# alexandre01/deepsvg

Hardware: AMD Instinct MI355X
Metric: SVG icons/sec (train step) hierarchical_ordered d=256 (higher is better)
Workload: dtype bf16; 1 GPU; hierarchical_ordered (Hierarchical, use_vae=False) G=8 S=30 d_model=256 ff=512 H=8 L=4x4; full train step = forward + SVGLoss + backward + grad-clip 1.0 + AdamW; dropout 0.1; global_batch=512, batch_per_gpu=512, parallelism=dp1, hip_graph=True, encoder_layout=packed (valid tokens only, exact)

## Files before the change

### deepsvg_amd/functional.py

```python
import math
import contextlib
import functools
import os

import torch

from . import ops

FFN_BWD_FUSED = os.environ.get("DSVG_FFN_BWD_FUSED", "0") != "0"
FFN_MIN_ROWS = int(os.environ.get("DSVG_FFN_MIN_ROWS", "16384"))
ATTN_MIN_ROWS = int(os.environ.get("DSVG_ATTN_MIN_ROWS", "16384"))
FFN_BWD_ORDER = os.environ.get("DSVG_FFN_BWD_ORDER", "1") != "0"
FFN_BWD_MASKED = int(os.environ.get("DSVG_FFN_BWD_MASKED", "0"))

GROUP_WGRAD = os.environ.get("DSVG_GROUP_WGRAD", "1") != "0"
BCAST_MASKED = os.environ.get("DSVG_BCAST_MASKED", "1") != "0"
LN_BWD_MASKED = os.environ.get("DSVG_LN_BWD_MASKED", "1") != "0"
DEFER_MORE = os.environ.get("DSVG_DEFER_MORE", "1") != "0"
STACK_GROUP = os.environ.get("DSVG_STACK_GROUP", "1") != "0"
STACK_GROUP_SLICES = int(os.environ.get("DSVG_STACK_GROUP_SLICES", "8"))
GS_BWD_DG = os.environ.get("DSVG_GS_BWD_DG", "1") != "0"
HEAD_KPAD = os.environ.get("DSVG_HEAD_KPAD", "1") != "0"
COND_GRAD_SHARED = os.environ.get("DSVG_COND_GRAD_SHARED", "1") != "0"
GS_STACK = os.environ.get("DSVG_GS_STACK", "1") != "0"
ATTN_BWD_OUTPROJ = os.environ.get("DSVG_ATTN_BWD_OUTPROJ", "1") != "0"
_ATTN_VALU = os.environ.get("DSVG_ATTN_VALU") is not None
_ATTN_MFMA_MIN_S = int(os.environ.get("DSVG_ATTN_MFMA_MIN_S", "2"))
ATTN_BWD_DX = os.environ.get("DSVG_ATTN_BWD_DX", "0") != "0"
ATTN_BWD_DX_MIN_ROWS = int(os.environ.get("DSVG_ATTN_BWD_DX_MIN_ROWS", "8192"))
GS_REMAINDER = int(os.environ.get("DSVG_GS_REMAINDER", "512"))
SEQ_ROUND = 2048
HEAD_FUSED = os.environ.get("DSVG_HEAD_FUSED", "0") != "0"

_NULL_CTX = contextlib.nullcontext()

class Runtime:

    def __init__(self, dtype=torch.float32, seed=None, store=None, training=False, defer=False):
        self.dtype = dtype
        self.defer = bool(defer)
        self.seed = seed
        self.store = store
        self.training = training
        self.masked = {}
        self.last_layer_gs = False
        self.stack_group = None
        self.cond_grad = {}

    def cond_grad_block(self, z, rows):
        if not COND_GRAD_SHARED or z is None or z.dim() != 2 or z.stride(1) != 1 or z.dtype != torch.bfloat16:
            return None
        w, ld = z.shape[1], z.stride(0)
        if ld <= w or ld % w or w % 8 or w > 512:
            return None
        i = (z.storage_offset() % ld) // w
        if (z.storage_offset() % ld) % w:
            return None
        base = z.data_ptr() - i * w * z.element_size()
        key = (base, rows, ld)
        buf = self.cond_grad.get(key)
        if buf is None:
            if len(self.cond_grad) > 8:
                self.cond_grad.clear()
            buf = self.cond_grad[key] = torch.empty((rows, ld), dtype=z.dtype, device=z.device)
        return buf[:, i * w:(i + 1) * w]

# ... 680 lines not shown
                elif ctx.needs_input_grad[3]:
                    dz = ops.gemm(dg, rt.w(wg), b_kc=False)
            nsl = STACK_GROUP_SLICES if (STACK_GROUP and GROUP_WGRAD and rt.defer) else 8
            gb = (lambda w_: nsl * -(-w_.shape[0] // 128) * -(-w_.shape[1] // 128)) if GROUP_WGRAD else (lambda w_: None)
            keep = rt.stack_group_begin() if (STACK_GROUP and GROUP_WGRAD and rt.defer) else None
            with (rt.grouping() if keep is None else _NULL_CTX):
                with ops.tag("ffn"):
                    dw2, db2 = _wbgrad(rt, w2, b2, dym, h, gb(w2))
                    dw1, db1 = _wbgrad(rt, w1, b1, dpre, xn2, gb(w1))
                if z is not None and wg is not None:
                    dwg, dbg = _wbgrad(rt, wg, bg, dg, z, gb(wg))
                dwo, dbo = _wbgrad(rt, wo, bo, dx1m, ao, gb(wo))
                dwin, dbin = _wbgrad(rt, win, bin_, dqkv, xn1, gb(win))
            if keep is not None:
                keep += [dym, h, dpre, xn2, dx1m, ao, dqkv, xn1, dg, z]
                if ctx.first_in_stack:
                    rt.stack_group_end()
            return (None, dx, None, dz, None, None, None, None, None, None,
                    dn1w, dn1b, dwin, dbin, dwo, dbo, dn2w, dn2b, dw1, db1, dw2, db2, dwg, dbg, None, None, None, None, None,
                    None, None, None)
        if ctx.ffn_fused:
            pb, b1f, w2p = rt.store.ffn(w1)[1:]
            T = x1.shape[0]
            with ops.tag("ffn"):
                g2p = torch.empty((256, 512), dtype=torch.float32, device=x1.device)
                g1p = torch.empty((512, 256), dtype=torch.float32, device=x1.device)
                db1p = torch.empty(512, dtype=torch.float32, device=x1.device)
                db2 = rt.grad_out(b2)
                s2, s1 = ops.split_k_for(256, 512, T), ops.split_k_for(512, 256, T)

                def wgrad2(dym, hp):
                    with rt.deferring():
                        if s2 > 1:
                            ops.gemm(dym, hp, a_kc=False, b_kc=False, out=g2p, split_k=s2, rowsum=db2)
                        else:
                            ops.gemm(dym, hp, a_kc=False, b_kc=False, out=g2p)
                            ops.colsum(dym, out=db2)

                def wgrad1(dpre, xh):
                    with rt.deferring():
                        if s1 > 1:
                            ops.gemm(dpre, xh, a_kc=False, b_kc=False, out=g1p, split_k=s1, rowsum=db1p)
                        else:
                            ops.gemm(dpre, xh, a_kc=False, b_kc=False, out=g1p)
                            ops.colsum(dpre, out=db1p)

                if h is None:
                    dx1, hp, dpre, xh, dym = ops.ffn_bwd(x1, dx2, pb, b1f, 1e-5, p, s0 + 3, s0 + 4, rt.seed)
                    wgrad2(dym, hp)
                    wgrad1(dpre, xh)
                else:
                    hp, xh = h, xn2
                    dym = dx2_masked if dx2_masked is not None else ops.drop_apply(dx2, p, s0 + 4, rt.seed)
                    if FFN_BWD_ORDER:
                        wgrad2(dym, hp)
                    dpre = ops.gemm(dym, w2p, b_kc=False, gate=hp, gate_scale=inv_keep)
                    if FFN_BWD_ORDER:
                        wgrad1(dpre, xh)
                    if FFN_BWD_MASKED == 1 or (FFN_BWD_MASKED == 2 and z is None and p > 0):
                        dx1, dx1m = ops.ffn_bwd_dx(dpre, x1, dx2, pb, masked=(p, s0 + 1, rt.seed))
                    else:
                        dx1 = ops.ffn_bwd_dx(dpre, x1, dx2, pb)
                    if not FFN_BWD_ORDER:
                        wgrad2(dym, hp)
                        wgrad1(dpre, xh)
                dw1, db1, dw2 = rt.grad_out(w1), rt.grad_out(b1), rt.grad_out(w2)
                dn2w, dn2b = rt.grad_out(n2w), rt.grad_out(n2b)
                fin = (g1p, db1p, g2p, w1.detach(), n2w.detach(), n2b.detach(), dw1.detach(), db1.detach(), dw2.detach(),
                       dn2w.detach(), dn2b.detach())
                if rt.defer:
                    ops.ffn_wgrad_finish_deferred(*fin)
                else:
                    ops.ffn_wgrad_finish(*fin)
            del hp, dpre, xh, dym
        else:
            with ops.tag("ffn"):
                dx2m = dx2_masked if dx2_masked is not None else ops.drop_apply(dx2, p, s0 + 4, rt.seed)
                dw2, db2 = _wbgrad(rt, w2, b2, dx2m, h)
                dh = ops.gemm(dx2m, rt.w(w2), b_kc=False, gate=h, gate_scale=inv_keep)
                dw1, db1 = _wbgrad(rt, w1, b1, dh, xn2)
                dxn2 = ops.gemm(dh, rt.w(w1), b_kc=False)
                with rt.deferring():
                    dx1, dn2w, dn2b = ops.layernorm_bwd(dxn2, x1, mean2, rstd2, n2w.detach(), res=dx2,
                                                        dgamma=rt.grad_out(n2w), dbeta=rt.grad_out(n2b))
            del dx2m
        dz = dl = dwg = dbg = dwg2 = dbg2 = None
        if l is not None:
            dg2 = ops.bcast_add_bwd(dx1, n_seq, S, p, s0 + 5, rt.seed)
            dwg2, dbg2 = _wbgrad(rt, wg2, bg2, dg2, l)
            if ctx.needs_input_grad[4]:
                dl = ops.gemm(dg2, rt.w(wg2), b_kc=False)
        if z is not None:
            vec = dx1.dtype == torch.bfloat16 and dx1.is_contiguous() and dx1.shape[1] % 8 == 0 and dx1.shape[1] <= 512
            dg_out = rt.cond_grad_block(z, n_seq_full) if (wg is None and vec and dx1.data_ptr() % 16 == 0) else None
            if BCAST_MASKED and dx1m is None and p > 0 and vec and n_seq * S <= dx1.shape[0] <= n_seq_full * S:
                dg, dx1m = ops.bcast_add_bwd(dx1, n_seq, S, p, s0 + 2, rt.seed, n_seq_out=n_seq_full, mask_site=s0 + 1, out=dg_out)
            else:
                dg = ops.bcast_add_bwd(dx1, n_seq, S, p, s0 + 2, rt.seed, n_seq_out=n_seq_full, out=dg_out)
            if wg is None:
                dz = dg
            else:
                dwg, dbg = _wbgrad(rt, wg, bg, dg, z)
                if ctx.needs_input_grad[3]:
                    dz = ops.gemm(dg, rt.w(wg), b_kc=False)
        if dx1m is None:
            dx1m = ops.drop_apply(dx1, p, s0 + 1, rt.seed)
        dwo, dbo = _wbgrad(rt, wo, bo, dx1m, ao)
        wob = None
        if (ATTN_BWD_OUTPROJ and not _ATTN_VALU and S >= _ATTN_MFMA_MIN_S
# ... 280 lines not shown
```

### deepsvg_amd/lib.py

```python
import ctypes as C
import os

_HERE = os.path.dirname(os.path.abspath(__file__))
LIB_PATH = os.path.join(_HERE, "_lib", "libdsvg_hip.so")

DSVG_F32 = 0
DSVG_BF16 = 1
ABI_VERSION = 9

c_i32, c_i64, c_u32, c_f32 = C.c_int32, C.c_int64, C.c_uint32, C.c_float
vp = C.c_void_p


class GemmDesc(C.Structure):
    _fields_ = [
        ("dtype", c_i32), ("M", c_i32), ("N", c_i32), ("K", c_i32),
        ("A", vp), ("lda", c_i64), ("a_kc", c_i32),
        ("B", vp), ("ldb", c_i64), ("b_kc", c_i32),
        ("C", vp), ("ldc", c_i64), ("c_f32", c_i32),
        ("bias", vp),
        ("res", vp), ("ldres", c_i64), ("res_pre", c_i32),
        ("act", c_i32),
        ("gate", vp), ("ldgate", c_i64), ("gate_scale", c_f32),
        ("drop_p", c_f32), ("drop_site", c_u32),
        ("a_drop_p", c_f32), ("a_drop_site", c_u32), ("a_drop_ld", c_i64),
        ("seed", vp),
        ("accumulate", c_i32),
        ("split_k", c_i32), ("workspace", vp), ("workspace_bytes", c_i64),
        ("rowsum", vp),
        ("impl", c_i32),
    ]


class GsFwdLayer(C.Structure):
    _fields_ = [(n, vp) for n in ("packed_fwd_layer", "in_bias", "out_bias", "b1", "b2", "gamma1", "beta1", "gamma2", "beta2",
                                  "seq_add", "x2", "mean1", "rstd1", "xn1", "qkv", "ao", "x1", "mean2", "rstd2", "xn2", "h")] + [
        ("site0", c_u32), ("reserved_", c_u32)]


class GsBwdLayer(C.Structure):
    _fields_ = [(n, vp) for n in ("packed_bwd_layer", "x", "mean1", "rstd1", "qkv", "x1", "mean2", "rstd2", "h", "gamma1", "gamma2",
                                  "dx", "dx1", "dym", "dpre", "dx1m", "dqkv", "dg", "dgamma2", "dbeta2", "dgamma1", "dbeta1",
                                  "workspace")] + [("site0", c_u32), ("reserved_", c_u32)]


SIGNATURES = {
    "dsvg_last_error": (C.c_char_p, []),
    "dsvg_version": (c_i32, []),
    "dsvg_gemm": (c_i32, [C.POINTER(GemmDesc), vp]),
    "dsvg_gemm_workspace_bytes": (c_i64, [c_i32, c_i32, c_i32]),
    "dsvg_reduce_partials": (c_i32, [vp, c_i64, c_i64, vp, c_i32, vp]),
    "dsvg_defer_scope": (c_i32, [c_i32, vp]),
    "dsvg_flush_deferred": (c_i32, [vp]),
    "dsvg_defer_zero": (c_i32, [vp, c_i64, vp]),
    "dsvg_gemm_group_scope": (c_i32, [c_i32, vp]),
    "dsvg_colsum": (c_i32, [c_i32, vp, c_i64, c_i64, c_i32, vp, c_i32, c_f32, c_u32, vp, vp, c_i64, vp]),
    "dsvg_colsum_workspace_bytes": (c_i64, [c_i64, c_i32]),
    "dsvg_layernorm_fwd": (c_i32, [c_i32, vp, vp, vp, vp, vp, vp, c_i64, c_i32, c_f32, vp]),
    "dsvg_layernorm_bwd": (c_i32, [c_i32, vp, vp, vp, vp, vp, vp, vp, vp, vp, c_i32, c_i64, c_i32, vp, c_i64, vp]),
    "dsvg_layernorm_bwd_workspace_bytes": (c_i64, [c_i64, c_i32]),
    "dsvg_layernorm_bwd_masked": (c_i32, [c_i32, vp, vp, vp, vp, vp, vp, vp, vp, vp, c_i32, c_i64, c_i32, vp, c_i64, vp, c_f32,
# ... 23 lines not shown
                                   c_i32, vp, c_i64, vp]),
    "dsvg_embed_scatter_workspace_bytes": (c_i64, [c_i64, c_i32, c_i32, c_i32, c_i32, c_i32, c_i32]),
    "dsvg_group_index": (c_i32, [vp, c_i64, c_i32, c_i32, vp, vp]),
    "dsvg_add_pos_fwd": (c_i32, [c_i32, vp, vp, vp, c_i64, c_i32, c_i32, c_f32, c_u32, vp, vp]),
    "dsvg_add_pos_bwd": (c_i32, [c_i32, vp, vp, vp, c_i32, c_i64, c_i32, c_i32, c_f32, c_u32, vp, vp, c_i64, vp]),
    "dsvg_add_pos_bwd_workspace_bytes": (c_i64, [c_i64, c_i32, c_i32]),
    "dsvg_masked_mean_fwd": (c_i32, [c_i32, vp, vp, vp, vp, c_i64, c_i32, c_i32, vp]),
    "dsvg_masked_mean_bwd": (c_i32, [c_i32, vp, vp, vp, c_i64, vp, c_i64, c_i32, c_i32, vp]),
    "dsvg_bcast_add_fwd": (c_i32, [c_i32, vp, vp, c_i64, c_i32, c_i32, c_f32, c_u32, vp, vp]),
    "dsvg_bcast_add_bwd": (c_i32, [c_i32, vp, vp, c_i64, c_i64, c_i32, c_i32, c_f32, c_u32, vp, c_i64, vp]),
    "dsvg_bcast_add_bwd_masked": (c_i32, [vp, vp, vp, c_i64, c_i64, c_i32, c_i32, c_i64, c_f32, c_u32, c_u32, vp, c_i64, vp]),
    "dsvg_loss_targets": (c_i32, [vp, vp, vp, c_i64, c_i32, c_i32, c_i32, c_i32, vp, vp, vp, vp, vp, vp, vp]),
    "dsvg_masked_ce_fwd": (c_i32, [c_i32, vp, c_i64, c_i32, vp, vp, c_i64, c_i32, vp, vp, vp, c_i64, vp, vp]),
    "dsvg_masked_ce_workspace_bytes": (c_i64, [c_i64]),
    "dsvg_masked_ce_bwd": (c_i32, [c_i32, vp, c_i64, c_i32, vp, vp, vp, vp, vp, c_f32, vp, c_i64, c_i64, c_i32, vp, c_i32, vp]),
    "dsvg_live_rows": (c_i32, [vp, c_i64, c_i32, vp, vp, vp, c_i64, vp]),
    "dsvg_live_rows_workspace_bytes": (c_i64, [c_i64]),
    "dsvg_scatter_rows": (c_i32, [c_i32, vp, vp, vp, c_i64, c_i32, c_i32, vp]),
    "dsvg_sumsq": (c_i32, [vp, c_i64, vp, vp, c_i64, vp]),
    "dsvg_sumsq_workspace_bytes": (c_i64, [c_i64]),
    "dsvg_adamw_step": (c_i32, [vp, vp, vp, vp, c_i64, vp, c_f32, c_f32, c_f32, c_f32, vp, vp, c_f32, c_f32, vp]),
    "dsvg_cast_weights": (c_i32, [c_i32, vp, vp, vp, c_i64, c_i64, vp]),
    "dsvg_advance_step": (c_i32, [vp, vp, vp]),
    "dsvg_pack_images": (c_i32, [vp, vp, c_i64, vp, c_i32, vp, vp, vp, vp, vp, c_i32, vp, vp, vp, c_i32, vp, vp, vp, vp, vp]),
    "dsvg_copy_many": (c_i32, [vp, vp, vp, c_i32, vp]),
    "dsvg_loss_combine_fwd": (c_i32, [vp, vp, c_i32, vp, vp]),
    "dsvg_loss_combine_bwd": (c_i32, [vp, vp, vp, c_i32, vp, vp]),
    "dsvg_gate_mul": (c_i32, [c_i32, vp, vp, vp, c_i64, c_f32, vp]),
    "dsvg_add": (c_i32, [c_i32, vp, vp, vp, c_i64, vp]),
    "dsvg_drop_apply": (c_i32, [c_i32, vp, vp, c_i64, c_f32, c_u32, vp, vp]),
    "dsvg_assemble_batch": (c_i32, [vp, c_i64, vp, c_i64, vp, c_i64, c_i32, c_i32, c_i32, c_f32, c_i32, vp, vp, vp,
                                    vp]),
    "dsvg_attention_causal_fwd": (c_i32, [c_i32, vp, vp, vp, c_i64, c_i32, c_i32, c_f32, c_f32, c_u32, vp, vp]),
    "dsvg_attention_causal_bwd": (c_i32, [c_i32, vp, vp, vp, vp, c_i64, c_i32, c_i32, c_f32, c_f32, c_u32, vp, vp]),
    "dsvg_seq_lens": (c_i32, [vp, c_i64, c_i32, c_i32, vp, vp]),
    "dsvg_attention_long_fwd": (c_i32, [c_i32, vp, vp, vp, c_i64, c_i32, c_i32, c_f32, c_i32, c_i32, c_f32, c_u32, vp,
                                        vp]),
    "dsvg_attention_long_bwd": (c_i32, [c_i32, vp, vp, vp, vp, c_i64, c_i32, c_i32, c_f32, c_i32, c_f32, c_u32, vp, vp]),
    "dsvg_prefix_mean_fwd": (c_i32, [c_i32, vp, vp, vp, c_i64, c_i32, c_i32, vp]),
    "dsvg_prefix_mean_bwd": (c_i32, [c_i32, vp, vp, vp, c_i64, c_i32, c_i32, vp]),
    "dsvg_match_costs": (c_i32, [c_i32, vp, c_i64, vp, c_i64, vp, c_i64, vp, vp, vp, c_i64, c_i32, c_i32, c_i32, c_i32,
                                 c_i32, c_i32, c_i32, c_f32, c_f32, c_f32, vp, vp, vp]),
    "dsvg_match_assign": (c_i32, [vp, vp, c_i64, c_i32, c_i32, vp, vp, vp, vp]),
    "dsvg_argmax_rows": (c_i32, [c_i32, vp, c_i64, c_i32, c_i64, c_i32, vp, vp]),
    "dsvg_sample_rows": (c_i32, [c_i32, vp, c_i64, c_i32, c_i64, c_i32, c_f32, vp, c_u32, vp, vp]),
    "dsvg_ffn_pack_bytes": (c_i64, [c_i32, c_i32]),
    "dsvg_ffn_pack": (c_i32, [vp, vp, c_i32, c_i32, c_i32, vp, vp, vp, vp, vp]),
    "dsvg_ffn_fwd": (c_i32, [vp, vp, vp, vp, vp, vp, vp, vp, c_i64, c_f32, c_f32, c_u32, c_u32, vp, c_i32, vp]),
    "dsvg_ffn_bwd": (c_i32, [vp, vp, vp, vp, vp, vp, vp, vp, vp, c_i64, c_f32, c_f32, c_u32, c_u32, vp, vp]),
    "dsvg_attn_bwd_dx_workspace_bytes": (c_i64, [c_i64]),
    "dsvg_attn_bwd_dx_debug_clock": (c_i32, [vp]),
    "dsvg_attn_bwd_dx": (c_i32, [vp, vp, vp, vp, vp, vp, vp, vp, vp, vp, c_i32, c_i64, vp, c_i64, vp, c_f32, c_u32, vp, vp]),
    "dsvg_ffn_bwd_dx": (c_i32, [vp, vp, vp, vp, vp, c_i64, c_f32, vp, c_f32, c_u32, vp, vp]),
    "dsvg_ffn_wgrad_finish": (c_i32, [vp] * 12),
    "dsvg_probe_trread": (c_i32, [vp, vp, vp]),
    "dsvg_attn_pack_bytes": (c_i64, [c_i32]),
    "dsvg_attn_pack": (c_i32, [vp, vp, c_i32, c_i32, c_i32, vp, vp]),
    "dsvg_attn_block_fwd": (c_i32, [vp, vp, vp, vp, vp, vp, vp, vp, vp, c_i64, c_i32, c_i64, vp, vp, vp, vp, vp, vp,
                                    c_f32, c_f32, c_f32, c_u32, c_u32, vp, vp, c_i64, c_u32, vp]),
    "dsvg_gs_pack_bytes": (c_i64, [c_i32]),
    "dsvg_gs_pack": (c_i32, [vp, vp, c_i32, c_i32, c_i32, c_i32, vp, vp, vp]),
    "dsvg_gs_layer_fwd": (c_i32, [vp] * 12 + [c_i64, c_i64, c_i32] + [vp] * 11 + [c_f32, c_f32, c_f32, c_u32, vp, c_i64, c_i32, vp]),
    "dsvg_gs_bwd_workspace_bytes": (c_i64, [c_i64, c_i32]),
    "dsvg_latent_chain_fwd": (c_i32, [vp, vp, vp, c_i32, vp, vp, vp, c_i64, vp]),
    "dsvg_latent_chain_bwd": (c_i32, [vp, vp, vp, c_i32, vp, vp, c_i64, vp]),
    "dsvg_gs_layer_bwd": (c_i32, [vp] * 13 + [c_i64, c_i32] + [vp] * 10 + [c_f32, c_f32, c_u32, vp, vp, c_i64, vp, vp]),
    "dsvg_gs_stack_fwd": (c_i32, [vp, vp, c_i32, vp, c_i64, c_i64, c_i32, c_f32, c_f32, c_f32, vp, vp]),
    "dsvg_gs_stack_bwd": (c_i32, [vp, vp, c_i32, vp, c_i64, c_i32, c_f32, c_f32, vp, c_i64, c_i64, vp]),
}

_lib = None


class DsvgError(RuntimeError):
    pass


def load():
    global _lib
    if _lib is not None:
        return _lib
    if not os.path.exists(LIB_PATH):
        raise DsvgError(
            f"{LIB_PATH} not found: the HIP extension is not built. Run `python -c \"import __graft_entry__ as g; "
            f"g.build()\"` (needs hipcc); there is no CPU fallback for the product path.")
    lib = C.CDLL(LIB_PATH)
    for name, (res, args) in SIGNATURES.items():
        fn = getattr(lib, name)
        fn.restype = res
        fn.argtypes = args
    built = lib.dsvg_version()
    if built != ABI_VERSION:
        raise DsvgError(f"{LIB_PATH} was built with DSVG_ABI_VERSION {built}, this binding expects {ABI_VERSION}: rebuild "
                        f"the library (deepsvg_amd/csrc/build.sh)")
    _lib = lib
    return lib


def check(rc, what):
    if rc != 0:
        msg = load().dsvg_last_error()
        raise DsvgError(f"{what} failed (rc={rc}): {msg.decode() if msg else '?'}")
```

### deepsvg_amd/ops.py

```python
import ctypes as C
import os

import torch

from . import lib as _l

F32, BF16 = _l.DSVG_F32, _l.DSVG_BF16
RELU = 1

PROFILE_ON = False
PROFILE = []
PROFILE_KEEP_DEFER = False
_TAG = None


def _event():
    return torch.cuda.Event(enable_timing=True)


class tag:

    def __init__(self, name):
        self.name = name

# ... 1047 lines not shown
        else:
            h = torch.empty((rows, 512), dtype=x.dtype, device=x.device)
            xh = torch.empty_like(x)
        rstd = torch.empty(rows, dtype=torch.float32, device=x.device)
    ev = _prof_begin()
    _l.check(_l.load().dsvg_ffn_fwd(x.data_ptr(), packed_fwd_layer.data_ptr(), b1f.data_ptr(), b2.data_ptr(),
                                    out.data_ptr(), _p(h), _p(xh), _p(rstd), rows, float(eps), float(drop_p),
                                    int(site_hidden), int(site_res), _p(seed) if drop_p > 0 else None,
                                    _FFN_STAGES if stages is None else int(stages), _stream()), "dsvg_ffn_fwd")
    _prof_end(ev, 4.0 * 256 * 512 * rows, (2.0 * 512 + (1536.0 if train else 0.0)) * rows, dict(op="ffn_fwd", rows=rows))
    return (out, h, xh, rstd) if train else out


def ffn_bwd(x, dy, packed_bwd_layer, b1f, eps=1e-5, drop_p=0.0, site_hidden=0, site_res=0, seed=None):
    _chk(x, dy, packed_bwd_layer, b1f, seed)
    assert x.dtype == torch.bfloat16 and x.dim() == 2 and x.shape[1] == 256 and x.is_contiguous()
    assert dy.dtype == x.dtype and dy.shape == x.shape and dy.is_contiguous()
    assert packed_bwd_layer.numel() == FFN_BWD_LAYER_ELEMS and packed_bwd_layer.is_contiguous() and b1f.numel() == 512
    rows = x.shape[0]
    dx, xh = torch.empty_like(x), torch.empty_like(x)
    dym = torch.empty_like(x) if drop_p > 0 else dy
    h = torch.empty((rows, 512), dtype=x.dtype, device=x.device)
    dpre = torch.empty((rows, 512), dtype=x.dtype, device=x.device)
    ev = _prof_begin()
    _l.check(_l.load().dsvg_ffn_bwd(x.data_ptr(), dy.data_ptr(), packed_bwd_layer.data_ptr(), b1f.data_ptr(),
                                    h.data_ptr(), dpre.data_ptr(), xh.data_ptr(), dym.data_ptr() if drop_p > 0 else None,
                                    dx.data_ptr(), rows, float(eps), float(drop_p), int(site_hidden), int(site_res),
                                    _p(seed) if drop_p > 0 else None, _stream()), "dsvg_ffn_bwd")
    _prof_end(ev, 4.0 * 256 * 512 * rows, (3 * 512 + 3 * 1024 + 512 + (512 if drop_p > 0 else 0)) * float(rows),
              dict(op="ffn_bwd", rows=rows))
    return dx, h, dpre, xh, dym


def ffn_bwd_dx(dpre, x, dy, packed_bwd_layer, eps=1e-5, masked=None):
    _chk(dpre, x, dy, packed_bwd_layer)
    assert x.dtype == torch.bfloat16 and x.dim() == 2 and x.shape[1] == 256 and x.is_contiguous()
    assert dy.dtype == x.dtype and dy.shape == x.shape and dy.is_contiguous()
    assert dpre.dtype == x.dtype and tuple(dpre.shape) == (x.shape[0], 512) and dpre.is_contiguous()
    assert packed_bwd_layer.numel() == FFN_BWD_LAYER_ELEMS and packed_bwd_layer.is_contiguous()
    dx = torch.empty_like(x)
    dxm, mp, msite, mseed = None, 0.0, 0, None
    if masked is not None and masked[0] > 0:
        mp, msite, mseed = float(masked[0]), int(masked[1]), masked[2]
        _chk(mseed)
        dxm = torch.empty_like(x)
    ev = _prof_begin()
    _l.check(_l.load().dsvg_ffn_bwd_dx(dpre.data_ptr(), x.data_ptr(), dy.data_ptr(), packed_bwd_layer.data_ptr(),
                                       dx.data_ptr(), x.shape[0], float(eps), _p(dxm), mp, msite, _p(mseed), _stream()),
             "dsvg_ffn_bwd_dx")
    _prof_end(ev, 2.0 * 256 * 512 * x.shape[0], (1024.0 + 3 * 512) * x.shape[0], dict(op="ffn_bwd_dx", rows=x.shape[0]))
    if masked is not None:
        return dx, (dxm if dxm is not None else dx)
    return dx


def ffn_wgrad_finish(g1p, db1p, g2p, w1, gamma, beta, dw1, db1, dw2, dgamma, dbeta):
    ts = (g1p, db1p, g2p, w1, gamma, beta, dw1, db1, dw2, dgamma, dbeta)
    _chk(*ts)
    assert all(t.dtype == torch.float32 and t.is_contiguous() for t in ts)
    assert g1p.numel() == 131072 and g2p.numel() == 131072 and db1p.numel() == 512 and w1.numel() == 131072
    assert dw1.numel() == 131072 and dw2.numel() == 131072 and db1.numel() == 512 and dgamma.numel() == 256
    assert dbeta.numel() == 256 and gamma.numel() == 256 and beta.numel() == 256
    ev = _prof_begin()
    _l.check(_l.load().dsvg_ffn_wgrad_finish(*(t.data_ptr() for t in ts), _stream()), "dsvg_ffn_wgrad_finish")
    _prof_end(ev, 0.0, 0.0, dict(op="ffn_wgrad_finish"))


def ffn_wgrad_finish_many(layers):
    if not layers:
        return
    flat = [t for ts in layers for t in ts]
    _chk(*flat)
    assert all(len(ts) == 11 for ts in layers) and all(t.dtype == torch.float32 and t.is_contiguous() for t in flat)
    ptrs = (C.c_void_p * len(flat))(*[t.data_ptr() for t in flat])
    ev = _prof_begin()
    _l.check(_l.load().dsvg_ffn_wgrad_finish_many(ptrs, len(layers), _stream()), "dsvg_ffn_wgrad_finish_many")
    _prof_end(ev, 0.0, 0.0, dict(op="ffn_wgrad_finish"))


def ffn_wgrad_finish_deferred(*ts):
    st = _DEFER.state.get(_stream_key())
    if st is None:
        ffn_wgrad_finish(*ts)
    else:
        st.finish.append(ts)


ATTN_LAYER_ELEMS = 512 * 512


def attn_pack(flat, offs, n_layers, packed=None):
    _chk(flat, offs, packed)
    assert flat.dtype == torch.float32 and offs.dtype == torch.int64 and tuple(offs.shape) == (n_layers, 2)
    assert offs.is_contiguous()
    if packed is None:
        packed = torch.empty(n_layers * ATTN_LAYER_ELEMS, dtype=torch.bfloat16, device=flat.device)
    assert packed.numel() == n_layers * ATTN_LAYER_ELEMS and packed.dtype == torch.bfloat16
    _l.check(_l.load().dsvg_attn_pack(flat.data_ptr(), offs.data_ptr(), n_layers, 256, 8, packed.data_ptr(), _stream()),
             "dsvg_attn_pack")
    return packed


def attn_block_fwd(x, packed_layer, in_bias, out_bias, gamma, beta, key_mask, n_seq, S, scale, eps=1e-5, drop_p=0.0,
                   site_probs=0, site_res=0, seed=None, seq_off=None, tiles=None, train=False, seq_add=None, site_seq_add=0,
                   into=None):
    _chk(x, packed_layer, in_bias, out_bias, gamma, beta, key_mask, seed, seq_off, tiles)
# ... 376 lines not shown
```

### include/dsvg.h

```cpp
#ifndef DSVG_H
#define DSVG_H

#include <stdint.h>
#include <stddef.h>

#ifdef __cplusplus
extern "C" {
#endif

#define DSVG_F32 0
#define DSVG_BF16 1

#define DSVG_ABI_VERSION 9

const char* dsvg_last_error(void);
int dsvg_version(void);

typedef struct dsvg_gemm_desc {
    int32_t dtype;
    int32_t M, N, K;
    const void* A; int64_t lda; int32_t a_kc;
    const void* B; int64_t ldb; int32_t b_kc;
    void* C; int64_t ldc; int32_t c_f32;
    const float* bias;
    const void* res; int64_t ldres; int32_t res_pre;
    int32_t act;
    const void* gate; int64_t ldgate; float gate_scale;
    float drop_p; uint32_t drop_site;
    float a_drop_p; uint32_t a_drop_site; int64_t a_drop_ld;
    const uint64_t* seed;
    int32_t accumulate;
    int32_t split_k; float* workspace; int64_t workspace_bytes;
    float* rowsum;
    int32_t impl;
} dsvg_gemm_desc;

int dsvg_gemm(const dsvg_gemm_desc* d, void* stream);
int64_t dsvg_gemm_workspace_bytes(int32_t M, int32_t N, int32_t split_k);

int dsvg_reduce_partials(const float* partial, int64_t P, int64_t n, float* out, int32_t accumulate,
                         void* stream);

int dsvg_defer_scope(int32_t on, void* stream);
int dsvg_defer_zero(float* out, int64_t n, void* stream);
int dsvg_flush_deferred(void* stream);
int dsvg_gemm_group_scope(int32_t on, void* stream);

int dsvg_colsum(int32_t dtype, const void* A, int64_t lda, int64_t M, int32_t N, float* out,
                int32_t accumulate, float drop_p, uint32_t drop_site, const uint64_t* seed,
                float* workspace, int64_t workspace_bytes, void* stream);
int64_t dsvg_colsum_workspace_bytes(int64_t M, int32_t N);

int dsvg_layernorm_fwd(int32_t dtype, const void* x, const float* gamma, const float* beta, void* y,
                       float* mean, float* rstd, int64_t rows, int32_t d, float eps, void* stream);
int dsvg_layernorm_bwd(int32_t dtype, const void* dy, const void* x, const float* mean,
                       const float* rstd, const float* gamma, const void* res, void* dx,
                       float* dgamma, float* dbeta, int32_t accumulate, int64_t rows, int32_t d,
                       float* workspace, int64_t workspace_bytes, void* stream);
int64_t dsvg_layernorm_bwd_workspace_bytes(int64_t rows, int32_t d);
int dsvg_layernorm_bwd_masked(int32_t dtype, const void* dy, const void* x, const float* mean, const float* rstd,
                              const float* gamma, const void* res, void* dx, float* dgamma, float* dbeta,
                              int32_t accumulate, int64_t rows, int32_t d, float* workspace, int64_t workspace_bytes,
                              void* dx_masked, float drop_p, uint32_t drop_site, const void* seed, void* stream);

int dsvg_attention_fwd(int32_t dtype, const void* qkv, const uint64_t* key_mask, const int32_t* seq_off,
                       int64_t total_rows, const int32_t* tile_first, void* out, int64_t n_seq, int32_t S,
// ... 115 lines not shown
                            uint32_t drop_site, const uint64_t* seed, void* stream);
int dsvg_attention_long_bwd(int32_t dtype, const void* qkv, const int32_t* seq_len, const void* dout, void* dqkv,
                            int64_t n_seq, int32_t S, int32_t n_heads, float scale, int32_t causal, float drop_p,
                            uint32_t drop_site, const uint64_t* seed, void* stream);
int dsvg_prefix_mean_fwd(int32_t dtype, const void* x, const int32_t* lens, void* out, int64_t n_seq, int32_t S, int32_t d,
                         void* stream);
int dsvg_prefix_mean_bwd(int32_t dtype, const void* dout, const int32_t* lens, void* dx, int64_t n_seq, int32_t S,
                         int32_t d, void* stream);

int dsvg_match_costs(int32_t dtype, const void* cmd_logits, int64_t ld_c, const void* args_logits, int64_t ld_a,
                     const void* vis_logits, int64_t ld_v, const float* tgt_commands, const float* tgt_args,
                     const float* cmd_args_mask, int64_t N, int32_t G, int32_t Gp, int32_t S1, int32_t n_args,
                     int32_t args_dim, int32_t n_cmd, int32_t eos_id, float w_args, float w_cmd, float w_vis,
                     float* cost, int32_t* visible, void* stream);
int dsvg_match_assign(const float* cost, const int32_t* visible, int64_t N, int32_t G, int32_t Gp,
                      int32_t* assign, int32_t* idx, int32_t* inv, void* stream);

int dsvg_argmax_rows(int32_t dtype, const void* logits, int64_t ld, int32_t group, int64_t rows, int32_t C,
                     int32_t* out, void* stream);
int dsvg_sample_rows(int32_t dtype, const void* logits, int64_t ld, int32_t group, int64_t rows, int32_t C,
                     float temperature, const void* seed, uint32_t site, int32_t* out, void* stream);

int64_t dsvg_head_pack_elems(int32_t n_out);
int dsvg_head_pack(const void* weight_bf16, int32_t n_out, void* packed, void* stream);
int dsvg_head_argmax(const void* x, const void* packed, const float* bias, int64_t rows, int32_t n_out, int32_t C,
                     int32_t* out_idx, void* stream);
int dsvg_head_sample(const void* x, const void* packed, const float* bias, int64_t rows, int32_t n_out, int32_t C,
                     float temperature, const void* seed, uint32_t site, int32_t* out_idx, void* stream);
int64_t dsvg_head_lse_workspace_bytes(int64_t rows);
int dsvg_head_lse(const void* x, const void* packed, const float* bias, int64_t rows, int32_t n_out, int32_t C,
                  const int32_t* target, const float* w, const int32_t* tok_idx, float* lse, float* sum_count,
                  float* workspace, int64_t workspace_bytes, void* stream);
int dsvg_head_dlogits(const void* x, const void* packed, const float* bias, int64_t rows, int32_t n_out, int32_t C,
                      const int32_t* target, const float* w, const int32_t* tok_idx, const float* lse,
                      const float* sum_count, const float* gscale, float coef, void* dlogits, int64_t ld_d, void* stream);

int dsvg_assemble_batch(const int16_t* rows, int64_t n_rows, const int32_t* slot_off, int64_t n_slots,
                        const int32_t* variant, int64_t n_items, int32_t G, int32_t grouped, int32_t L,
                        float pad_val, int32_t args_dim, float* commands, float* args, float* args_rel,
                        void* stream);

int64_t dsvg_ffn_pack_bytes(int32_t n_layers, int32_t which);
int dsvg_ffn_pack(const float* flat_f32, const int64_t* offs, int32_t n_layers, int32_t d_model, int32_t d_ff,
                  void* packed_fwd, void* packed_bwd, float* b1_folded, void* w2p, void* stream);
int dsvg_ffn_fwd(const void* x, const void* packed_fwd_layer, const float* b1_folded, const float* b2, void* y,
                 void* h_out, void* xh_out, float* rstd_out, int64_t rows, float eps, float drop_p,
                 uint32_t site_hidden, uint32_t site_res, const void* seed, int32_t stages, void* stream);
int dsvg_ffn_bwd(const void* x, const void* dy, const void* packed_bwd_layer, const float* b1_folded, void* h, void* dpre,
                 void* xh, void* dym, void* dx, int64_t rows, float eps, float drop_p, uint32_t site_hidden,
                 uint32_t site_res, const void* seed, void* stream);
int dsvg_ffn_bwd_dx(const void* dpre, const void* x, const void* dy, const void* packed_bwd_layer, void* dx,
                    int64_t rows, float eps, void* dx_masked, float drop_p, uint32_t drop_site, const void* seed,
                    void* stream);
int dsvg_ffn_wgrad_finish(const float* g1p, const float* db1p, const float* g2p, const float* w1, const float* gamma,
                          const float* beta, float* dw1, float* db1, float* dw2, float* dgamma, float* dbeta,
                          void* stream);
int dsvg_ffn_wgrad_finish_many(const void* const* ptrs, int32_t n_layers, void* stream);
int dsvg_ffn_debug_clock(void* buf);
int dsvg_gs_debug_clock(void* buf);

int64_t dsvg_attn_pack_bytes(int32_t n_layers);
int dsvg_attn_pack(const float* flat_f32, const int64_t* offs, int32_t n_layers, int32_t d_model, int32_t n_heads,
                   void* packed, void* stream);
int dsvg_attn_block_fwd(const void* x, const void* packed_layer, const float* in_bias, const float* out_bias,
                        const float* gamma, const float* beta, const uint64_t* key_mask, const int32_t* seq_off,
                        const int32_t* tile_first, int64_t n_seq, int32_t S, int64_t rows, void* x1, void* xn_out,
                        void* qkv_out, void* ao_out, float* mean_out, float* rstd_out, float eps, float scale,
                        float drop_p, uint32_t site_probs, uint32_t site_res, const void* seed,
                        const void* seq_add, int64_t seq_add_ld, uint32_t site_seq_add, void* stream);
int64_t dsvg_gs_pack_bytes(int32_t n_layers);
int dsvg_gs_pack(const float* flat_f32, const int64_t* offs, int32_t n_layers, int32_t d_model, int32_t d_ff,
                 int32_t n_heads, void* packed_fwd, void* packed_bwd, void* stream);
int dsvg_gs_layer_fwd(const void* x, const void* packed_fwd_layer, const float* in_bias, const float* out_bias,
                      const float* b1, const float* b2, const float* gamma1, const float* beta1, const float* gamma2,
                      const float* beta2, const uint64_t* key_mask, const void* seq_add, int64_t seq_add_ld, int64_t n_seq, int32_t S,
                      void* x2, float* mean1, float* rstd1, void* xn1, void* qkv, void* ao, void* x1, float* mean2,
                      float* rstd2, void* xn2, void* h, float eps, float scale, float drop_p, uint32_t site0,
                      const void* seed, int64_t seq_base, int32_t ffn_format, void* stream);
int64_t dsvg_gs_bwd_workspace_bytes(int64_t n_seq, int32_t S);
int dsvg_gs_layer_bwd(const void* dx2, const void* packed_bwd_layer, const void* x, const float* mean1, const float* rstd1,
                      const void* qkv, const void* x1, const float* mean2, const float* rstd2, const void* h,
                      const float* gamma1, const float* gamma2, const uint64_t* key_mask, int64_t n_seq, int32_t S,
                      void* dx, void* dx1, void* dym, void* dpre, void* dx1m, void* dqkv, float* dgamma2, float* dbeta2,
                      float* dgamma1, float* dbeta1, float scale, float drop_p, uint32_t site0, const void* seed,
                      void* workspace, int64_t workspace_bytes, void* dg, void* stream);
typedef struct dsvg_gs_fwd_layer {
    const void* packed_fwd_layer;
    const float *in_bias, *out_bias, *b1, *b2, *gamma1, *beta1, *gamma2, *beta2;
    const void* seq_add;
    void* x2;
    float *mean1, *rstd1;
    void *xn1, *qkv, *ao, *x1;
    float *mean2, *rstd2;
    void *xn2, *h;
    uint32_t site0;
    uint32_t reserved_;
} dsvg_gs_fwd_layer;
typedef struct dsvg_gs_bwd_layer {
    const void* packed_bwd_layer;
    const void* x;
    const float *mean1, *rstd1;
    const void *qkv, *x1;
    const float *mean2, *rstd2;
    const void* h;
    const float *gamma1, *gamma2;
    void *dx, *dx1, *dym, *dpre, *dx1m, *dqkv, *dg;
// ... 23 lines not shown
```

Before: 90810 icons/s.

## Fuse FFN gated dgrad GEMM with W2 weight-gradient split-K GEMM sharing dym/hp tiles

Adds a HIP kernel that loads each 64-row tile of dym and hp into LDS once and uses it for two jobs. Half the waves compute the gated dpre = (dym·W2)⊙relu'(hp)·scale, and the other half accumulate split-K partials of dW2 = dymᵀ·hp plus the db2 row sums. This replaces two separate kernels that each streamed dym and hp from memory. The cost is a more intricate kernel with triple-buffered DMA loads, and an imbalance between the two wave groups that could leave CUs idle.

```diff
diff --git a/deepsvg_amd/csrc/ffn_bwd_gate.hip b/deepsvg_amd/csrc/ffn_bwd_gate.hip
--- /dev/null
+++ b/deepsvg_amd/csrc/ffn_bwd_gate.hip
@@ -0,0 +1,351 @@
+#include <stdlib.h>
+#include "dsvg_common.h"
+#include "../../include/dsvg.h"
+
+typedef __bf16 bf16x8 __attribute__((ext_vector_type(8)));
+typedef short shortx4 __attribute__((ext_vector_type(4)));
+typedef float floatx16 __attribute__((ext_vector_type(16)));
+
+namespace {
+
+constexpr int GT = 64;
+constexpr int W2_BYTES = 256 * 64 * 2;
+constexpr int SLOT = (2 * 64 * 128 + 64 * 64) * 2;
+constexpr int HP_OFF = 2 * 64 * 128 * 2;
+constexpr int NSLOT = 3;
+constexpr int LDS_BYTES = W2_BYTES + NSLOT * SLOT;
+static_assert(LDS_BYTES <= 160 * 1024, "LDS budget of a CU");
+
+#define DSVG_LDS_PTR(p) ((void __attribute__((address_space(3)))*)(p))
+
+union Frag8 {
+    bf16x8 v;
+    shortx4 h[2];
+    uint4 u;
+};
+
+__device__ __forceinline__ int sw256(int r) { return ((r & 3) << 2) | ((r >> 2) & 3); }
+__device__ __forceinline__ int sw128(int r) { return ((r >> 1) & 1) << 2; }
+
+__device__ __forceinline__ void dma5(const char* s0, const char* s1, const char* s2, const char* s3, const char* s4,
+                                     uint32_t lds) {
+    uint32_t keep;
+    asm volatile(
+        "s_mov_b32 %0, m0\n\t"
+        "s_mov_b32 m0, %6\n\t"
+        "s_nop 0\n\t"
+        "global_load_lds_dwordx4 %1, off\n\t"
+        "s_add_u32 m0, m0, 0x400\n\t"
+        "s_nop 0\n\t"
+        "global_load_lds_dwordx4 %2, off\n\t"
+        "s_add_u32 m0, m0, 0x400\n\t"
+        "s_nop 0\n\t"
+        "global_load_lds_dwordx4 %3, off\n\t"
+        "s_add_u32 m0, m0, 0x400\n\t"
+        "s_nop 0\n\t"
+        "global_load_lds_dwordx4 %4, off\n\t"
+        "s_add_u32 m0, m0, 0x400\n\t"
+        "s_nop 0\n\t"
+        "global_load_lds_dwordx4 %5, off\n\t"
+        "s_mov_b32 m0, %0"
+        : "=&s"(keep)
+        : "v"(s0), "v"(s1), "v"(s2), "v"(s3), "v"(s4), "s"(lds)
+        : "memory", "scc");
+}
+__device__ __forceinline__ void dma4(const char* s0, const char* s1, const char* s2, const char* s3, uint32_t lds) {
+    uint32_t keep;
+    asm volatile(
+        "s_mov_b32 %0, m0\n\t"
+        "s_mov_b32 m0, %5\n\t"
+        "s_nop 0\n\t"
+        "global_load_lds_dwordx4 %1, off\n\t"
+        "s_add_u32 m0, m0, 0x400\n\t"
+        "s_nop 0\n\t"
+        "global_load_lds_dwordx4 %2, off\n\t"
+        "s_add_u32 m0, m0, 0x400\n\t"
+        "s_nop 0\n\t"
+        "global_load_lds_dwordx4 %3, off\n\t"
+        "s_add_u32 m0, m0, 0x400\n\t"
+        "s_nop 0\n\t"
+        "global_load_lds_dwordx4 %4, off\n\t"
+        "s_mov_b32 m0, %0"
+        : "=&s"(keep)
+        : "v"(s0), "v"(s1), "v"(s2), "v"(s3), "s"(lds)
+        : "memory", "scc");
+}
+
+__device__ __forceinline__ bf16x8 ld_tr(const char* img, uint32_t off0, uint32_t off1) {
+    Frag8 f;
+    f.h[0] = __builtin_amdgcn_ds_read_tr16_b64_v4i16((shortx4 __attribute__((address_space(3)))*)(img + off0));
+    f.h[1] = __builtin_amdgcn_ds_read_tr16_b64_v4i16((shortx4 __attribute__((address_space(3)))*)(img + off1));
+    return f.v;
+}
+
+__device__ __forceinline__ bf16x8 zero_from(const bf16x8& v, int lim) {
+    Frag8 f;
+    f.v = v;
+    uint32_t w[4] = {f.u.x, f.u.y, f.u.z, f.u.w};
+#pragma unroll
+    for (int e = 0; e < 4; ++e) w[e] = 2 * e >= lim ? 0u : (2 * e + 1 >= lim ? (w[e] & 0xffffu) : w[e]);
+    f.u = make_uint4(w[0], w[1], w[2], w[3]);
+    return f.v;
+}
+
+__device__ __forceinline__ float rowsum8(const bf16x8& f, float s) {
+    typedef __bf16 bf16x2 __attribute__((ext_vector_type(2)));
+    Frag8 t;
+    t.v = f;
+    const uint32_t w[4] = {t.u.x, t.u.y, t.u.z, t.u.w};
+    const bf16x2 one = __builtin_bit_cast(bf16x2, 0x3f803f80u);
+#pragma unroll
+    for (int e = 0; e < 4; ++e) s = __builtin_amdgcn_fdot2_f32_bf16(__builtin_bit_cast(bf16x2, w[e]), one, s, false);
+    return s;
+}
+
+__global__ __launch_bounds__(512, 1) void ffn_gate_dw2_kernel(const bf16_t* __restrict__ dym, const bf16_t* __restrict__ hp,
+                                                               const bf16_t* __restrict__ w2p, float gate_scale,
+                                                               bf16_t* __restrict__ dpre, int T, int k_chunk, int xcd_map,
+                                                               float* __restrict__ part, int part_bf16) {
+    extern __shared__ __attribute__((aligned(1024))) char lds[];
+    const int bid = (int)blockIdx.x;
+    int c, z;
+    if (xcd_map) { const int local = bid >> 3; c = local & 7; z = (local >> 3) * 8 + (bid & 7); }
+    else { c = bid & 7; z = bid >> 3; }
+    const int row_begin = z * k_chunk;
+    const int row_end = min(T, row_begin + k_chunk);
+    const int n_tiles = row_end > row_begin ? (row_end - row_begin + GT - 1) / GT : 0;
+
+    const int tid = threadIdx.x, lane = tid & 63;
+    const int wave = __builtin_amdgcn_readfirstlane(tid >> 6);
+    const int h = lane >> 5;
+    const uint32_t lds0 = (uint32_t)(uintptr_t)DSVG_LDS_PTR(lds);
+
+    const char* src[5];
+    int srow[5];
+    long long sld[5];
+#pragma unroll
+    for (int i = 0; i < 5; ++i) {
+        const int P = wave * 5 + i;
+        if (P < 32) {
+            const int r = 4 * (P & 15) + (lane >> 4);
+            const int ch = (lane & 15) ^ sw256(r);
+            src[i] = (const char*)dym + (size_t)(128 * (P >> 4) + 8 * ch) * 2;
+            srow[i] = r;
+            sld[i] = 256 * 2;
+        } else {
+            const int r = 8 * (P - 32) + (lane >> 3);
+            const int ch = (lane & 7) ^ sw128(r);
+            src[i] = (const char*)hp + (size_t)(64 * c + 8 * ch) * 2;
+            srow[i] = r;
+            sld[i] = 512 * 2;
+        }
+    }
+    auto issue = [&](int s) {
+        const int r0 = row_begin + s * GT;
+        const char* a[5];
+#pragma unroll
+        for (int i = 0; i < 5; ++i) a[i] = src[i] + (size_t)min(r0 + srow[i], T - 1) * sld[i];
+        const uint32_t dst = __builtin_amdgcn_readfirstlane(lds0 + W2_BYTES + (uint32_t)(s % NSLOT) * SLOT + (uint32_t)wave * 5 * 1024);
+        dma5(a[0], a[1], a[2], a[3], a[4], dst);
+    };
+
+    const int g = lane >> 4, q = lane & 15, qq = q >> 2, pp = q & 3;
+    const bool p1 = wave < 4;
+    const int wm = (wave >> 1) & 1, wn = wave & 1;
+    const int ww = wave & 3;
+    const int trow = 8 * (g >> 1) + qq;
+    const int pr = 32 * wm + (lane & 31);
+    const uint32_t w2_off = (uint32_t)(trow * 128 + 16 * ((4 * wn + 2 * (g & 1) + (pp >> 1)) ^ sw128(trow)) + 8 * (pp & 1));
+    uint32_t da_off[2][2], hb_off[2];
+#pragma unroll
+    for (int it = 0; it < 2; ++it)
+#pragma unroll
+        for (int sc = 0; sc < 2; ++sc) {
+            const int r = trow + 4 * sc;
+            const int ch = 8 * (ww & 1) + 4 * it + 2 * (g & 1) + (pp >> 1);
+            da_off[it][sc] = (uint32_t)((ww >> 1) * 16384 + r * 256 + 16 * (ch ^ sw256(r)) + 8 * (pp & 1));
+        }
+#pragma unroll
+    for (int jn = 0; jn < 2; ++jn)
+        hb_off[jn] = (uint32_t)(HP_OFF + trow * 128 + 16 * ((4 * jn + 2 * (g & 1) + (pp >> 1)) ^ sw128(trow)) + 8 * (pp & 1));
+
+    floatx16 acc00, acc01, acc10, acc11;
+#pragma unroll
+    for (int r = 0; r < 16; ++r) { acc00[r] = 0.f; acc01[r] = 0.f; acc10[r] = 0.f; acc11[r] = 0.f; }
+    const bool do_rs = !p1 && c == 0;
+    float rsa0 = 0.f, rsa1 = 0.f, rsb0 = 0.f, rsb1 = 0.f;
+
+    auto compute = [&](int s) {
+        const char* slot = lds + W2_BYTES + (s % NSLOT) * SLOT;
+        const int r0 = row_begin + s * GT;
+        if (p1) {
+            floatx16 acc;
+#pragma unroll
+            for (int r = 0; r < 16; ++r) acc[r] = 0.f;
+#pragma unroll
+            for (int kk = 0; kk < 16; ++kk) {
+                Frag8 a;
+                a.u = *reinterpret_cast<const uint4*>(slot + (kk >> 3) * 16384 + pr * 256 +
+                                                      16 * ((2 * (kk & 7) + h) ^ sw256(pr)));
+                const bf16x8 b = ld_tr(lds, w2_off + kk * 2048, w2_off + kk * 2048 + 512);
+                acc = __builtin_amdgcn_mfma_f32_32x32x16_bf16(b, a.v, acc, 0, 0, 0);
+            }
+            uint32_t x[4][4];
+#pragma unroll
+            for (int gq = 0; gq < 4; ++gq)
+#pragma unroll
+                for (int e = 0; e < 4; ++e) x[gq][e] = __float_as_uint(acc[4 * gq + e]);
+#pragma unroll
+            for (int e = 0; e < 4; ++e) {
+                auto s01 = __builtin_amdgcn_permlane32_swap(x[0][e], x[1][e], false, false);
+                auto s23 = __builtin_amdgcn_permlane32_swap(x[2][e], x[3][e], false, false);
+                x[0][e] = s01[0]; x[1][e] = s01[1]; x[2][e] = s23[0]; x[3][e] = s23[1];
+            }
+#pragma unroll
+            for (int e = 0; e < 4; ++e) {
+                auto s02 = __builtin_amdgcn_permlane32_swap(x[0][e], x[2][e], false, false);
+                auto s13 = __builtin_amdgcn_permlane32_swap(x[1][e], x[3][e], false, false);
+                x[0][e] = s02[0]; x[2][e] = s02[1]; x[1][e] = s13[0]; x[3][e] = s13[1];
+            }
+            uint4 pk[2];
+#pragma unroll
+            for (int cb = 0; cb < 2; ++cb) {
+                float v[8];
+#pragma unroll
+                for (int e = 0; e < 4; ++e) { v[e] = __uint_as_float(x[2 * cb][e]); v[4 + e] = __uint_as_float(x[2 * cb + 1][e]); }
+                const uint4 gt = *reinterpret_cast<const uint4*>(slot + HP_OFF + pr * 128 +
+                                                                 16 * ((4 * wn + 2 * h + cb) ^ sw128(pr)));
+                const uint32_t gw[4] = {gt.x, gt.y, gt.z, gt.w};
+#pragma unroll
+                for (int e = 0; e < 4; ++e) {
+                    const float g0 = __uint_as_float(gw[e] << 16), g1 = __uint_as_float(gw[e] & 0xffff0000u);
+                    v[2 * e] = g0 > 0.f ? v[2 * e] * gate_scale : 0.f;
+                    v[2 * e + 1] = g1 > 0.f ? v[2 * e + 1] * gate_scale : 0.f;
+                }
+                pk[cb] = make_uint4(f2bf_pk(v[0], v[1]), f2bf_pk(v[2], v[3]), f2bf_pk(v[4], v[5]), f2bf_pk(v[6], v[7]));
+            }
+            const int m = r0 + pr;
+            if (m < row_end) {
+                bf16_t* cp = dpre + (size_t)m * 512 + 64 * c + 32 * wn + 16 * h;
+                *reinterpret_cast<uint4*>(cp) = pk[0];
+                *reinterpret_cast<uint4*>(cp + 8) = pk[1];
+            }
+        } else {
+            const bool ragged = r0 + GT > row_end;
+#pragma unroll
+            for (int kk = 0; kk < 4; ++kk) {
+                bf16x8 a0 = ld_tr(slot, da_off[0][0] + kk * 4096, da_off[0][1] + kk * 4096);
+                bf16x8 a1 = ld_tr(slot, da_off[1][0] + kk * 4096, da_off[1][1] + kk * 4096);
+                const bf16x8 b0 = ld_tr(slot, hb_off[0] + kk * 2048, hb_off[0] + kk * 2048 + 512);
+                const bf16x8 b1 = ld_tr(slot, hb_off[1] + kk * 2048, hb_off[1] + kk * 2048 + 512);
+                if (ragged) {
+                    const int lim = row_end - (r0 + 16 * kk + 8 * h);
+                    a0 = zero_from(a0, lim);
+                    a1 = zero_from(a1, lim);
+                }
+                acc00 = __builtin_amdgcn_mfma_f32_32x32x16_bf16(b0, a0, acc00, 0, 0, 0);
+                acc01 = __builtin_amdgcn_mfma_f32_32x32x16_bf16(b0, a1, acc01, 0, 0, 0);
+                acc10 = __builtin_amdgcn_mfma_f32_32x32x16_bf16(b1, a0, acc10, 0, 0, 0);
+                acc11 = __builtin_amdgcn_mfma_f32_32x32x16_bf16(b1, a1, acc11, 0, 0, 0);
+                if (do_rs) {
+                    if (kk < 2) { rsa0 = rowsum8(a0, rsa0); rsa1 = rowsum8(a1, rsa1); }
+                    else { rsb0 = rowsum8(a0, rsb0); rsb1 = rowsum8(a1, rsb1); }
+                }
+            }
+        }
+    };
+
+    if (n_tiles > 0) {
+        const char* a[4];
+#pragma unroll
+        for (int i = 0; i < 4; ++i) {
+            const int r = 8 * (wave * 4 + i) + (lane >> 3);
+            const int ch = (lane & 7) ^ sw128(r);
+            a[i] = (const char*)w2p + ((size_t)r * 512 + 64 * c + 8 * ch) * 2;
+        }
+        dma4(a[0], a[1], a[2], a[3], __builtin_amdgcn_readfirstlane(lds0 + (uint32_t)wave * 4 * 1024));
+    }
+    for (int s = 0; s < 2 && s < n_tiles; ++s) issue(s);
+    for (int s = 0; s < n_tiles; ++s) {
+        if (s + 1 < n_tiles) asm volatile("s_waitcnt vmcnt(5)" ::: "memory");
+        else asm volatile("s_waitcnt vmcnt(0)" ::: "memory");
+        __builtin_amdgcn_s_barrier();
+        if (s + 2 < n_tiles) issue(s + 2);
+        compute(s);
+    }
+    if (p1) return;
+
+    const size_t slice = dsvg_splitk_slice(256, 512, true);
+    float* my_part = part + (size_t)z * slice;
+    const int mrow = 64 * ww + (lane & 31);
+    const int ncol = 64 * c;
+    auto put = [&](const floatx16& v, int jn, int im) {
+        const int m = mrow + 32 * im;
+#pragma unroll
+        for (int gq = 0; gq < 4; ++gq) {
+            const int n = ncol + 32 * jn + 8 * gq + 4 * h;
+            *reinterpret_cast<float4*>(my_part + (size_t)m * 512 + n) = make_float4(v[4 * gq], v[4 * gq + 1], v[4 * gq + 2], v[4 * gq + 3]);
+        }
+    };
+    auto put_bf16 = [&](const floatx16& v, int jn, int im) {
+        const int m = mrow + 32 * im;
+        bf16_t* base = reinterpret_cast<bf16_t*>(my_part);
+#pragma unroll
+        for (int gp = 0; gp < 2; ++gp) {
+            const uint32_t a0 = f2bf_pk(v[8 * gp + 0], v[8 * gp + 1]), a1 = f2bf_pk(v[8 * gp + 2], v[8 * gp + 3]);
+            const uint32_t b0 = f2bf_pk(v[8 * gp + 4], v[8 * gp + 5]), b1 = f2bf_pk(v[8 * gp + 6], v[8 * gp + 7]);
+            auto s0 = __builtin_amdgcn_permlane32_swap(a0, b0, false, false);
+            auto s1 = __builtin_amdgcn_permlane32_swap(a1, b1, false, false);
+            const int n = ncol + 32 * jn + 16 * gp + 8 * h;
+            *reinterpret_cast<uint4*>(base + (size_t)m * 512 + n) = make_uint4(s0[0], s1[0], s0[1], s1[1]);
+        }
+    };
+    if (part_bf16) { put_bf16(acc00, 0, 0); put_bf16(acc01, 0, 1); put_bf16(acc10, 1, 0); put_bf16(acc11, 1, 1); }
+    else { put(acc00, 0, 0); put(acc01, 0, 1); put(acc10, 1, 0); put(acc11, 1, 1); }
+    if (do_rs) {
+        rsa0 += __shfl_xor(rsa0, 32, 64);
+        rsa1 += __shfl_xor(rsa1, 32, 64);
+        rsb0 += __shfl_xor(rsb0, 32, 64);
+        rsb1 += __shfl_xor(rsb1, 32, 64);
+        if (h == 0) {
+            float* rs = my_part + 256 * 512;
+            rs[mrow] = rsa0 + rsb0;
+            rs[mrow + 32] = rsa1 + rsb1;
+        }
+    }
+}
+
+}
+
+extern "C" int dsvg_ffn_gate_dw2(const void* dym, const void* hp, const void* w2p, float gate_scale, void* dpre,
+                                 int64_t rows, int32_t split_k, float* g2p, float* db2, float* workspace,
+                                 int64_t workspace_bytes, void* stream) {
+    DSVG_CHECK_ARG(dym && hp && w2p && dpre && g2p && db2 && workspace, "ffn_gate_dw2: null operand");
+    DSVG_CHECK_ARG(rows > 0 && rows < (1ll << 30) && split_k > 1, "ffn_gate_dw2: bad rows %lld / split_k %d",
+                   (long long)rows, split_k);
+    DSVG_CHECK_ARG(workspace_bytes >= dsvg_gemm_workspace_bytes(256, 512, split_k), "ffn_gate_dw2: workspace too small");
+    DSVG_CHECK_ARG(!(((uintptr_t)dym | (uintptr_t)hp | (uintptr_t)w2p | (uintptr_t)dpre | (uintptr_t)workspace) & 15),
+                   "ffn_gate_dw2: operands must be 16-byte aligned");
+    static const bool pbf_on = !(getenv("DSVG_SPLITK_BF16") && atoi(getenv("DSVG_SPLITK_BF16")) == 0);
+    hipStream_t st = (hipStream_t)stream;
+    const int T = (int)rows;
+    const int k_chunk = ((T + split_k - 1) / split_k + 63) / 64 * 64;
+    int nsplit = (T + k_chunk - 1) / k_chunk;
+    if ((split_k % 8) == 0) nsplit = split_k;
+    const int pbf = (pbf_on && (T % 64) == 0) ? 1 : 0;
+    static bool once = false;
+    if (!once) {
+        (void)hipFuncSetAttribute((const void*)ffn_gate_dw2_kernel, hipFuncAttributeMaxDynamicSharedMemorySize, LDS_BYTES);
+        once = true;
+    }
+    hipLaunchKernelGGL(ffn_gate_dw2_kernel, dim3(8 * nsplit), dim3(512), LDS_BYTES, st, (const bf16_t*)dym,
+                       (const bf16_t*)hp, (const bf16_t*)w2p, gate_scale, (bf16_t*)dpre, T, k_chunk,
+                       (nsplit % 8) == 0 ? 1 : 0, workspace, pbf);
+    DSVG_LAUNCH_CHECK("ffn_gate_dw2");
+    const int64_t mn = 256 * 512;
+    const int64_t slice = (int64_t)dsvg_splitk_slice(256, 512, true);
+    int rc = pbf ? dsvg_reduce_partials_mixed(workspace, nsplit, slice, mn, mn, g2p, 0, st)
+                 : dsvg_reduce_partials_strided(workspace, nsplit, slice, mn, g2p, 0, st);
+    if (rc) return rc;
+    return dsvg_reduce_partials_strided(workspace + mn, nsplit, slice, 256, db2, 0, st);
+}
diff --git a/deepsvg_amd/functional.py b/deepsvg_amd/functional.py
--- a/deepsvg_amd/functional.py
+++ b/deepsvg_amd/functional.py
@@ -12,6 +12,7 @@
 ATTN_MIN_ROWS = int(os.environ.get("DSVG_ATTN_MIN_ROWS", "16384"))
 FFN_BWD_ORDER = os.environ.get("DSVG_FFN_BWD_ORDER", "1") != "0"
 FFN_BWD_MASKED = int(os.environ.get("DSVG_FFN_BWD_MASKED", "0"))
+FFN_GATE_DW2 = os.environ.get("DSVG_FFN_GATE_DW2", "1") != "0"
 
 GROUP_WGRAD = os.environ.get("DSVG_GROUP_WGRAD", "1") != "0"
 BCAST_MASKED = os.environ.get("DSVG_BCAST_MASKED", "1") != "0"
@@ -798,9 +799,14 @@
                 else:
                     hp, xh = h, xn2
                     dym = dx2_masked if dx2_masked is not None else ops.drop_apply(dx2, p, s0 + 4, rt.seed)
-                    if FFN_BWD_ORDER:
-                        wgrad2(dym, hp)
-                    dpre = ops.gemm(dym, w2p, b_kc=False, gate=hp, gate_scale=inv_keep)
+                    if (FFN_GATE_DW2 and FFN_BWD_ORDER and s2 > 1 and dym.is_cuda and dym.dtype == torch.bfloat16
+                            and dym.is_contiguous() and hp.is_contiguous() and w2p.is_contiguous()):
+                        with rt.deferring():
+                            dpre = ops.ffn_gate_dw2(dym, hp, w2p, inv_keep, g2p, db2, s2)
+                    else:
+                        if FFN_BWD_ORDER:
+                            wgrad2(dym, hp)
+                        dpre = ops.gemm(dym, w2p, b_kc=False, gate=hp, gate_scale=inv_keep)
                     if FFN_BWD_ORDER:
                         wgrad1(dpre, xh)
                     if FFN_BWD_MASKED == 1 or (FFN_BWD_MASKED == 2 and z is None and p > 0):
diff --git a/deepsvg_amd/lib.py b/deepsvg_amd/lib.py
--- a/deepsvg_amd/lib.py
+++ b/deepsvg_amd/lib.py
@@ -6,7 +6,7 @@
 
 DSVG_F32 = 0
 DSVG_BF16 = 1
-ABI_VERSION = 9
+ABI_VERSION = 10
 
 c_i32, c_i64, c_u32, c_f32 = C.c_int32, C.c_int64, C.c_uint32, C.c_float
 vp = C.c_void_p
@@ -136,6 +136,7 @@
     "dsvg_attn_bwd_dx_debug_clock": (c_i32, [vp]),
     "dsvg_attn_bwd_dx": (c_i32, [vp, vp, vp, vp, vp, vp, vp, vp, vp, vp, c_i32, c_i64, vp, c_i64, vp, c_f32, c_u32, vp, vp]),
     "dsvg_ffn_bwd_dx": (c_i32, [vp, vp, vp, vp, vp, c_i64, c_f32, vp, c_f32, c_u32, vp, vp]),
+    "dsvg_ffn_gate_dw2": (c_i32, [vp, vp, vp, c_f32, vp, c_i64, c_i32, vp, vp, vp, c_i64, vp]),
     "dsvg_ffn_wgrad_finish": (c_i32, [vp] * 12),
     "dsvg_probe_trread": (c_i32, [vp, vp, vp]),
     "dsvg_attn_pack_bytes": (c_i64, [c_i32]),
diff --git a/deepsvg_amd/ops.py b/deepsvg_amd/ops.py
--- a/deepsvg_amd/ops.py
+++ b/deepsvg_amd/ops.py
@@ -1123,6 +1123,26 @@
     if masked is not None:
         return dx, (dxm if dxm is not None else dx)
     return dx
+
+
+def ffn_gate_dw2(dym, hp, w2p, gate_scale, g2p, db2, split_k):
+    _chk(dym, hp, w2p, g2p, db2)
+    T = dym.shape[0]
+    assert dym.dtype == torch.bfloat16 and dym.dim() == 2 and dym.shape[1] == 256 and dym.is_contiguous()
+    assert hp.dtype == dym.dtype and tuple(hp.shape) == (T, 512) and hp.is_contiguous()
+    assert w2p.dtype == dym.dtype and tuple(w2p.shape) == (256, 512) and w2p.is_contiguous()
+    assert g2p.dtype == torch.float32 and g2p.numel() == 131072 and g2p.is_contiguous()
+    assert db2.dtype == torch.float32 and db2.numel() == 256 and db2.is_contiguous()
+    assert split_k > 1
+    L = _l.load()
+    dpre = torch.empty((T, 512), dtype=dym.dtype, device=dym.device)
+    ws = _ws(L.dsvg_gemm_workspace_bytes(256, 512, split_k), dym.device)
+    ev = _prof_begin()
+    _l.check(L.dsvg_ffn_gate_dw2(dym.data_ptr(), hp.data_ptr(), w2p.data_ptr(), float(gate_scale), dpre.data_ptr(), T,
+                                 int(split_k), g2p.data_ptr(), db2.data_ptr(), ws.data_ptr(), ws.numel() * 4, _stream()),
+             "dsvg_ffn_gate_dw2")
+    _prof_end(ev, 4.0 * 256 * 512 * T, 2.0 * (256 + 512 + 512) * T, dict(op="ffn_gate_dw2", rows=T))
+    return dpre
 
 
 def ffn_wgrad_finish(g1p, db1p, g2p, w1, gamma, beta, dw1, db1, dw2, dgamma, dbeta):
diff --git a/include/dsvg.h b/include/dsvg.h
--- a/include/dsvg.h
+++ b/include/dsvg.h
@@ -11,7 +11,7 @@
 #define DSVG_F32 0
 #define DSVG_BF16 1
 
-#define DSVG_ABI_VERSION 9
+#define DSVG_ABI_VERSION 10
 
 const char* dsvg_last_error(void);
 int dsvg_version(void);
@@ -233,6 +233,8 @@
 int dsvg_ffn_bwd_dx(const void* dpre, const void* x, const void* dy, const void* packed_bwd_layer, void* dx,
                     int64_t rows, float eps, void* dx_masked, float drop_p, uint32_t drop_site, const void* seed,
                     void* stream);
+int dsvg_ffn_gate_dw2(const void* dym, const void* hp, const void* w2p, float gate_scale, void* dpre, int64_t rows,
+                      int32_t split_k, float* g2p, float* db2, float* workspace, int64_t workspace_bytes, void* stream);
 int dsvg_ffn_wgrad_finish(const float* g1p, const float* db1p, const float* g2p, const float* w1, const float* gamma,
                           const float* beta, float* dw1, float* db1, float* dw2, float* dgamma, float* dbeta,
                           void* stream);
```

Measured after the change: 92570 icons/s (median of 6 runs). +1.9%, better.
